# MiZhenxing/Switch-NeRF

Measured on AMD Instinct MI355X. Metric: train rays/sec (8192-ray batch, 256 samples, 8 experts), higher is better.
Workload: dtype bf16; 1 GPU; configs[1]: 8-expert top-1 expertmlp, capacity_factor=1.0, BPR, 8192 rays x 256 samples per step over 1 GPU(s) (8192 rays per GPU), 16 segments of 131072 points per GPU, building.yaml shapes, random-init weights, gate_scale=1.0; global_batch_rays=8192, rays_per_gpu=8192, samples=256, segment_points=131072, parallelism=dp1

## Files before the change

### include/swn.h

```cpp
#ifndef SWN_H
#define SWN_H
#include <stddef.h>
#include <stdint.h>

#ifdef __cplusplus
extern "C" {
#endif

#define SWN_F32 0
#define SWN_BF16 1
#define SWN_F16 2

const char* swn_last_error(void);
int swn_version(void);
int swn_half_dtype(void);

int swn_mfma_probe(int32_t* out, void* stream);

int swn_sample_pe(const float* rays, const float* t_steps, const float* perturb_rand, float perturb,
                  int n_rays, int n_samples, int l_xyz, int l_dir, int dtype,
                  float* z_out, void* pe_xyz, int pe_stride, void* pe_dir, int dir_stride, void* stream);

#define SWN_RNG_UNIFORM 0
#define SWN_RNG_NORMAL 1
// ... 233 lines not shown
  const float* comb_dsig;
  const float* comb_wsig;
  const float* comb_gate;
  float* comb_dgate;
  float* comb_dwsig;
  float* comb_dwsig_ws;
  const float* heads_ws;
  const float* heads_bs;
  const float* heads_wc;
  const float* heads_bc;
  const float* heads_noise;
  float* heads_raw;
  int32_t* sched;
  int32_t x_features;
  int32_t x_k;
  int32_t head_layers;
  int32_t tail_first;
  int32_t y_features;
  const float* tail_gate;
  const int32_t* tail_dropped;
  const int32_t* tail_n_dropped;
  int32_t tail_dropped_max;
  int32_t tail_tokens;
  const int32_t* tail_bias_row;
  swn_chain_layer layers[SWN_MAX_CHAIN_LAYERS];
  int32_t packed_rows;
} swn_chain_desc;

int swn_mlp_chain(const swn_chain_desc* desc, void* stream);
size_t swn_chain_dwsig_workspace_bytes(int n_groups, int group_rows_clamp);
// ... 163 lines not shown
```

### switch_nerf_amd/_lib.py

```python
from __future__ import annotations

import ctypes as C
import os

_HERE = os.path.dirname(os.path.abspath(__file__))
LIB_PATH = os.environ.get("SWN_LIB") or os.path.join(_HERE, "libswn_hip.so")
LIB_PATH_F16 = os.path.join(_HERE, "libswn_hip_f16.so")

F32, BF16, F16 = 0, 1, 2


def source_hash() -> str:
    import hashlib
    h = hashlib.sha256()
    files = [os.path.join(_HERE, "csrc", f) for f in sorted(os.listdir(os.path.join(_HERE, "csrc")))]
    files += [os.path.join(os.path.dirname(_HERE), "include", "swn.h"), os.path.join(_HERE, "build.sh")]
    for f in files:
        if os.path.isfile(f):
            h.update(os.path.basename(f).encode() + b"\0")
            h.update(open(f, "rb").read())
    return h.hexdigest()

vp, i32, i64, f32, sz, u64 = C.c_void_p, C.c_int, C.c_long, C.c_float, C.c_size_t, C.c_uint64

# ... 20 lines not shown
    _fields_ = [("n_levels", i32), ("log2_table", i32), ("base_res", i32), ("per_level_scale", f32), ("aabb_lo", f32 * 3),
                ("aabb_hi", f32 * 3)]


class Camera(C.Structure):
    _fields_ = [("c2w", f32 * 12), ("fx", f32), ("fy", f32), ("cx", f32), ("cy", f32), ("W", C.c_int32), ("H", C.c_int32),
                ("center_pixels", C.c_int32), ("reserved", C.c_int32), ("image_index", C.c_int64)]


class ChainDesc(C.Structure):
    _fields_ = [("dtype", i32), ("n_layers", i32), ("n_groups", i32), ("n_wsets", i32), ("group_stride", i32),
                ("group_rows", vp), ("group_rows_clamp", i32), ("group_begin", vp), ("x", vp), ("x_gather", vp), ("x_save", vp), ("x_scale", vp), ("x_relu", i32),
                ("y", vp), ("y_add", vp), ("y_add_gather", vp), ("geometry", i32), ("tag", i32),
                ("comb_y", vp), ("comb_dsig", vp), ("comb_wsig", vp), ("comb_gate", vp), ("comb_dgate", vp), ("comb_dwsig", vp), ("comb_dwsig_ws", vp),
                ("heads_ws", vp), ("heads_bs", vp), ("heads_wc", vp), ("heads_bc", vp), ("heads_noise", vp), ("heads_raw", vp), ("sched", vp), ("x_features", i32),
                ("x_k", i32), ("head_layers", i32), ("tail_first", i32), ("y_features", i32), ("tail_gate", vp), ("tail_dropped", vp), ("tail_n_dropped", vp),
                ("tail_dropped_max", i32), ("tail_tokens", i32), ("tail_bias_row", vp),
                ("layers", ChainLayer * 12), ("packed_rows", i32)]


SIGNATURES = {
    "swn_version": [],
    "swn_mfma_probe": [vp, vp],
    "swn_sample_pe": [vp, vp, vp, f32, i32, i32, i32, i32, i32, vp, vp, i32, vp, i32, vp],
    "swn_sample_pe_rng": [vp, vp, u64, vp, i64, f32, i32, i32, i32, i32, i32, vp, vp, i32, vp, i32, vp],
    "swn_rng_fill": [vp, i64, i64, i32, f32, u64, vp, i32, vp],
    "swn_rng_fill_rows": [vp, i64, i64, i64, vp, i64, i32, f32, u64, vp, i32, i32, vp],
    "swn_rng_advance": [vp, vp],
    "swn_pe_from_z": [vp, vp, i32, i32, i32, i32, vp, i32, vp],
    "swn_sample_pdf": [vp, vp, vp, i32, i32, i32, vp, vp],
    "swn_cascade_resample": [vp, vp, vp, i32, i32, i32, vp, vp, vp],
# ... 180 lines not shown
```

### switch_nerf_amd/csrc/chain.hip

```cpp
#include "common.hpp"

#ifndef SWN_WIDE
#define SWN_WIDE 0
#endif
#ifndef SWN_CONCAT
#define SWN_CONCAT 0
#endif
#if SWN_WIDE == 2
#define SWN_NS swn_wide2
#elif SWN_WIDE
#define SWN_NS swn_wide
#elif SWN_CONCAT
#define SWN_NS swn_cat
#else
#define SWN_NS swn
#endif
#define SWN_AUX (SWN_WIDE || SWN_CONCAT)
#ifndef SWN_STATIC_EPI
#define SWN_STATIC_EPI 1
#endif
#if defined(SWN_EXP_TIMING) && (!SWN_AUX || SWN_WIDE == 2)
#define SWN_TIMING_ON 1
#else
#define SWN_TIMING_ON 0
// ... 1154 lines not shown
  SWN_CHECK(!d.comb_dwsig == !d.comb_dwsig_ws && (!d.comb_dwsig || (d.head_layers > 0 && d.comb_y && d.comb_dsig)),
            "swn_mlp_chain: comb_dwsig and comb_dwsig_ws come together, with the combine backward of a fused backward chain (head_layers > 0, comb_y, comb_dsig)");
  SWN_CHECK(d.tag != 8 || d.head_layers > 0, "swn_mlp_chain: tag 8 is the expert backward chain behind the tail's backward layers (head_layers > 0)");
  SWN_CHECK(d.tail_first == 0 || (d.geometry == 7 && d.tag == 7), "swn_mlp_chain: a fused tail (tail_first > 0) runs on geometry 7 with tag 7");
  SWN_CHECK(d.tag != 7 || d.tail_first > 0, "swn_mlp_chain: tag 7 is the fused-tail forward chain (tail_first > 0)");
  SWN_CHECK(d.x_features == 0 || d.x_features == d.layers[0].k || (d.x_features == 128 && d.layers[0].k == 256 && d.geometry >= 6),
            "swn_mlp_chain: x_features = %d: only 128-feature rows under a zero-padded k = 256 first layer on geometry 6 / 7", d.x_features);
  if (d.x_k != 0) {
    SWN_CHECK(d.x_k > 0 && d.x_k <= 256, "swn_mlp_chain: x_k = %d not in (0, 256]", d.x_k);
    SWN_CHECK(d.x_k % 16 == 0, "swn_mlp_chain: x_k = %d is not a multiple of the K step (16)", d.x_k);
    SWN_CHECK(d.geometry >= 6, "swn_mlp_chain: x_k = %d: only the persistent chains (geometry 6 / 7) take a real K, not geometry %d", d.x_k, d.geometry);
    SWN_CHECK(d.x_features == 128, "swn_mlp_chain: x_k = %d needs x_features = 128 (a first layer zero-padded in K), not %d", d.x_k, d.x_features);
    SWN_CHECK(d.x_k <= ((d.x_features + 15) & ~15), "swn_mlp_chain: x_k = %d beyond x_features = %d", d.x_k, d.x_features);
    SWN_CHECK(d.tail_first == 0, "swn_mlp_chain: x_k = %d: a fused tail's chain input is 256 features wide", d.x_k);
  }
  SWN_CHECK(!(wide && concat), "swn_mlp_chain: concat-skip layers are built for the 256-feature kernels only");
  SWN_CHECK(d.geometry >= 0 && d.geometry <= 7, "swn_mlp_chain: geometry %d not in [0,7]", d.geometry);
  SWN_CHECK(d.packed_rows >= 0, "swn_mlp_chain: packed_rows %d < 0", d.packed_rows);
  if (d.packed_rows > 0) {
    SWN_CHECK(d.group_begin != nullptr, "swn_mlp_chain: packed mask slots (packed_rows > 0) address the groups through group_begin");
    SWN_CHECK(d.geometry <= 1 || d.geometry == 7, "swn_mlp_chain: packed mask slots (packed_rows > 0) run on geometry 0 / 1 or 7, not %d",
              d.geometry);
  }
  if (d.comb_y && d.head_layers == 0) {
    const int nl = d.layers[d.n_layers - 1].n;
    SWN_CHECK(d.comb_gate && d.comb_dgate, "swn_mlp_chain: combine backward needs comb_gate and comb_dgate");
    SWN_CHECK((nl == 128 || nl == 256 || nl == 512) && nl * (d.dtype == SWN_F32 ? 4 : 2) <= 1024,
              "swn_mlp_chain: combine backward: last layer of 128 / 256 / 512 features, at most 1 KiB per row");
    SWN_CHECK((d.geometry < 2 || d.geometry >= 6) && (d.tag & 0xFF) == 5,
              "swn_mlp_chain: combine backward runs on the 64-row kernels (geometry 0 / 1) or the persistent ones (6 / 7), tag 5");
// ... 21 lines not shown
```

### switch_nerf_amd/csrc/chain_big.hip

```cpp
#include "common.hpp"

namespace swn_big {
using namespace swn;

typedef __attribute__((ext_vector_type(8))) short bf16x8_t;
typedef __attribute__((ext_vector_type(8))) _Float16 f16x8_t;
typedef __attribute__((ext_vector_type(4))) float f32x4_t;
typedef __attribute__((ext_vector_type(16))) float f32x16_t;
typedef __attribute__((ext_vector_type(4))) uint32_t u32x4_t;
typedef __attribute__((ext_vector_type(2))) uint32_t u32x2_t;
typedef __attribute__((ext_vector_type(2))) _Float16 f16x2_t;
#define SWN_LDS(p) ((__attribute__((address_space(3))) void*)(p))
#define SWN_GLB(p) ((const __attribute__((address_space(1))) void*)(p))

constexpr int ROWB = 512;
constexpr int SLOT_B = 8192;
constexpr int NSLOT = 3;
constexpr int KSTEPS = 16;

template <int NW_, int MI_> struct Geo {
  static constexpr int NW = NW_, MI = MI_;
  static constexpr int RG = NW / 4;
  static constexpr int BM = RG * MI * 32;
  static constexpr int NT = NW * 64;
// ... 523 lines not shown
    SWN_MM(1, 1);
    SWN_PIN();
    SWN_MM(2, 0);
    SWN_PIN();
    SWN_MM(2, 1);
    SWN_PIN();
    SWN_MM(3, 0);
    SWN_PIN();
    SWN_MM(3, 1);
#undef SWN_MM
    SWN_PIN();
  }
}
#endif

template <typename E, int RELU, bool BIAS, bool SKIP, typename HOOK>
__device__ __forceinline__ void epilogue_p(f32x16_t (&acc)[4][2], const Ctx& cx, u32x4_t& mk, int bias_off, HOOK hook) {
  typedef G256 G;
  char* smem = cx.smem;
  uint32_t e_base = cx.e_base, e2_base = cx.e2_base;
  asm volatile("" : "+v"(e_base), "+v"(e2_base));
  f32x4_t bias[2][4];
  if constexpr (BIAS) {
#pragma unroll
    for (int ni = 0; ni < 2; ++ni)
#pragma unroll
      for (int g4 = 0; g4 < 4; ++g4)
        bias[ni][g4] = *(const f32x4_t*)(smem + G::BIAS0 + bias_off + (((cx.w & 3) * 64 + 32 * ni + 8 * g4 + 4 * cx.lhi) << 2));
  }
#pragma unroll
// ... 640 lines not shown
      SWN_PIN();
#pragma unroll
      for (int g = 0; g < 4; g += 2) {
        auto r0 = __builtin_amdgcn_permlane32_swap(pp[g * 2], pp[(g + 1) * 2], false, false);
        auto r1 = __builtin_amdgcn_permlane32_swap(pp[g * 2 + 1], pp[(g + 1) * 2 + 1], false, false);
        const u32x4_t o = {(uint32_t)r0[0], (uint32_t)r1[0], (uint32_t)r0[1], (uint32_t)r1[1]};
        *(u32x4_t*)(smem + (e2_base ^ (uint32_t)((4 * ni + g) << 4)) + mi * (32 * ROWB)) = o;
      }
      SWN_PIN();
      if constexpr (hook_halves<HOOK>::value) hook(t);
      else if (t & 1) hook(t >> 1);
    }
  }
}

template <typename E, typename PRE>
__device__ __forceinline__ void write_rows128_tok(const Ctx& cx, void* y, uint32_t oob, const float* wc, int idx_off, int rows, bool heads, PRE pre,
                                                  u32x4_t (&keep)[16]) {
  char* smem = cx.smem;
  const int* idx = (const int*)(smem + idx_off);
  const int l15 = cx.lane & 15, rq = cx.lane >> 4;
  const int rbase = 128 * (cx.w >> 2) + 2 * (cx.w & 3) + 8 * (rq >> 1) + (rq & 1);
  const __amdgpu_buffer_rsrc_t rs = uniform_rsrc(y ? y : (void*)wc, y ? (int)oob : 0);
  f32x4_t w[3][2];
  if (heads) {
#pragma unroll
    for (int c = 0; c < 3; ++c)
#pragma unroll
      for (int q = 0; q < 2; ++q) w[c][q] = *(const f32x4_t*)(smem + T_WC + ((c * 128 + l15 * 8 + 4 * q) << 2));
  }
// ... 25 lines not shown
        a += __int_as_float(__builtin_amdgcn_update_dpp(0, __float_as_int(a), 0x4E, 0xF, 0xF, true));
        a += __int_as_float(__builtin_amdgcn_update_dpp(0, __float_as_int(a), 0x141, 0xF, 0xF, true));
        a += __int_as_float(__builtin_amdgcn_update_dpp(0, __float_as_int(a), 0x140, 0xF, 0xF, true));
        if (l15 == c) ((float*)(smem + T_COL))[c * 256 + rbase + 16 * i] = a;
      }
    }
  }
}

__device__ __forceinline__ int fresh_lane() {
  int l;
  asm volatile("v_mbcnt_lo_u32_b32 %0, -1, 0\n\tv_mbcnt_hi_u32_b32 %0, -1, %0" : "=v"(l));
  return l;
}

template <typename E, int TAG, bool BIAS_INIT, int XS>
__device__ __forceinline__ void chainq_body(const ArgsQ& args) {
  extern __shared__ __attribute__((aligned(16))) char smem[];
  typedef G256 G;
  constexpr int BM = G::BM, MI = 4;
  constexpr bool TAIL = TAG == 7;
  constexpr bool HEAD = TAG == 8;
  constexpr bool DROPS = TAIL || HEAD;
  const swn_chain_desc& d = args.d;
  Ctx cx;
  cx.smem = smem;
  const int tid = threadIdx.x;
  cx.lane = tid & 63;
  cx.w = __builtin_amdgcn_readfirstlane(tid >> 6);
  cx.l31 = cx.lane & 31;
  cx.lhi = cx.lane >> 5;
// ... 27 lines not shown
  auto claim = [&]() -> int {
    int q = 0;
    if (d.sched) {
      const int sq = cur_sq();
      if (fresh_lane() == 0) q = __hip_atomic_fetch_add(d.sched + ((xq + sq) & 7), 1, __ATOMIC_RELAXED, __HIP_MEMORY_SCOPE_AGENT);
    }
    return q;
  };
  auto next_queue = [&]() -> bool {
    int m = 0;
    int sq = cur_sq();
    const int bit = 1 << ((xq + sq) & 7);
    if (fresh_lane() == 0) m = __hip_atomic_fetch_or(d.sched + 9, bit, __ATOMIC_RELAXED, __HIP_MEMORY_SCOPE_AGENT) | bit;
    m = __builtin_amdgcn_readfirstlane(m);
    do { ++sq; } while (sq < 8 && ((m >> ((xq + sq) & 7)) & 1));
    if (fresh_lane() == 0) *(volatile int*)(gcount + 2) = sq;
    return sq < 8;
  };
  auto grab = [&](int slot, int ticket) {
    int vb, g = 0, tile = 0, rows_valid = 0;
    bool first = true;
    int n_groups = d.n_groups, tpg = args.tiles_per_group, n_wsets = d.n_wsets;
    asm volatile("" : "+s"(n_groups), "+s"(tpg), "+s"(n_wsets));
    for (;;) {
      int q;
      if (d.sched) {
        q = first ? ticket : claim();
        first = false;
        q = __builtin_amdgcn_readfirstlane(q);
        const int xs = (xq + cur_sq()) & 7;
        if (args.n_queues != 8) vb = q;
// ... 90 lines not shown
    if (lt < 128) {
      const int r = 128 * rg + lt;
      const long gr = t.grow0 + (r < t.rows ? r : 0);
      if ((TAIL && t.l0) || (HEAD && t.l1 < n_layers)) src = d.tail_dropped[gr];
      else src = d.x_gather ? d.x_gather[gr] : (int)gr;
    }
    return src;
  };
  auto store_row = [&](int src, int idx_off) {
    const int lt = fg * 64 + fresh_lane();
    if (lt < 128) ((int*)(smem + idx_off))[128 * rg + lt] = src < 0 ? 0 : src;
  };
  const bool narrow = d.x_features == 128;
  constexpr bool k_short = XS != KSTEPS;
  static_assert(!k_short || !TAIL, "a fused tail's chain input is 256 features wide");
  auto wrs = [&](int L, int wset) -> __amdgpu_buffer_rsrc_t {
    const int bytes = 8 * (d.layers[L].k >> 4) * 1024;
    const char* p = (const char*)d.layers[L].w + (size_t)wset * bytes;
    return uniform_rsrc(p, bytes);
  };
  auto ws_of = [&](int L, const Tile& t) -> int {
    return ((TAIL && L >= d.tail_first) || (HEAD && L < d.head_layers)) ? 0 : t.wset;
  };
  auto out_rs = [&](void* base, const Tile& t) -> __amdgpu_buffer_rsrc_t {
    return uniform_rsrc((char*)base + t.grow0 * ROWB, t.rows * ROWB);
  };
  u32x4_t wq[WQD][2];
  auto preload_w = [&](int L, int wset, int lane_) {
    const __amdgpu_buffer_rsrc_t r = wrs(L, wset);
#pragma unroll
    for (int ks = 0; ks < WQA; ++ks)
#pragma unroll
      for (int i = 0; i < 2; ++i) wq[ks][i] = __builtin_amdgcn_raw_buffer_load_b128(r, lane_ * 16, ((2 * fg + i) * (d.layers[L].k >> 4) + ks) * 1024, 0);
  };
  auto stage_bias = [&](int L, int wset, int slot) {
    const float* b = d.layers[L].b;
    if (b) {
      const __amdgpu_buffer_rsrc_t rb = uniform_rsrc(b + (size_t)wset * 256, 1024);
      __builtin_amdgcn_raw_ptr_buffer_load_lds(rb, SWN_LDS(smem + G::BIAS0 + slot * 1024 + fg * 256), 4, fresh_lane() * 4, fg * 256, 0, 0);
    } else if constexpr (BIAS_INIT) {
      *(float*)(smem + G::BIAS0 + slot * 1024 + fg * 256 + fresh_lane() * 4) = 0.f;
    }
  };
  auto load_mask = [&](int L, int vb) -> u32x4_t {
    const swn_chain_layer& l_ = d.layers[L];
    if (l_.relu == 2) return *(const u32x4_t*)(l_.mask + ((size_t)(vb * G::NW + cx.w) * 64 + fresh_lane()) * 4);
    return u32x4_t{0u, 0u, 0u, 0u};
  };
  constexpr bool bias_init = BIAS_INIT;
  f32x4_t bv[2][4];
  auto load_bv = [&](int slot) {
    if constexpr (BIAS_INIT) {
      const int lh_ = fresh_lane() >> 5;
#pragma unroll
      for (int ni = 0; ni < 2; ++ni)
#pragma unroll
        for (int g4 = 0; g4 < 4; ++g4)
          bv[ni][g4] = *(const f32x4_t*)(smem + G::BIAS0 + slot * 1024 + ((fg * 64 + 32 * ni + 8 * g4 + 4 * lh_) << 2));
    }
  };

  for (int i = ((int)(blockIdx.x >> 3) & 15) * args.stagger; i > 0; --i) __builtin_amdgcn_s_sleep(16);
  const int yf = TAIL ? (d.y_features ? d.y_features : 256) : 256;
  const uint32_t oob_y = (uint32_t)d.tail_tokens * (uint32_t)(yf * 2), oob_s = (uint32_t)d.tail_tokens * (uint32_t)ROWB;
  auto tail_out = [&](const Ctx& c_, const Tile& t, int idx_off, u32x4_t (&keep)[16]) {
    const bool hd = d.heads_raw != nullptr;
    const int r = 128 * (c_.w >> 2) + 8 * (c_.l31 >> 1) + 2 * (c_.w & 3) + (c_.l31 & 1);
    const bool fin = hd && c_.lhi == 0 && r < t.rows;
// ... 136 lines not shown
      if constexpr (HEAD) {
        if (cur.l1 == n_layers && lts < 128) {
          ((float*)(smem + T_GATE))[128 * rgs + lts] = gate_v;
          ((float*)(smem + T_DSIG))[128 * rgs + lts] = dsig_v;
        }
      }
    }
    if (rg == 0 && it == 0) { stage_bias(cur.l0, ws_of(cur.l0, cur), 0); SWN_WAIT_VM(0); }
    u32x4_t mk_next = load_mask(cur.l0, cur.vb);
    SWN_PIN();
    preload_w(cur.l0, ws_of(cur.l0, cur), fresh_lane());
    SWN_PIN();
    SWN_TM(const long long s1 = TICK(); tS += s1 - s0;)
    Tile nxt = cur;
    const int l_end = HEAD ? cur.l1 : n_layers;
    auto run_layer = [&](const int L, auto first_c) {
      constexpr bool SHORT_K = decltype(first_c)::value;
      const swn_chain_layer& ly = d.layers[L];
      const bool last = L + 1 == l_end;
      load_bv(bc % 3);
      SWN_PIN();
      SWN_WAIT_LGKM0();
      __builtin_amdgcn_s_barrier();
      u32x4_t mk = mk_next;
      if (last) nxt = read_tile((it + 1) & 1);
      {
        SWN_TM(const long long k0 = TICK();)
        const __amdgpu_buffer_rsrc_t rs_cur = wrs(L, ws_of(L, cur));
        if (rg == 0) {
          if (!last) stage_bias(L + 1, ws_of(L + 1, cur), (bc + 1) % 3);
          else if (nxt.vb >= 0) stage_bias(nxt.l0, ws_of(nxt.l0, nxt), (bc + 1) % 3);
        }
        if constexpr (bias_init) {
#pragma unroll
          for (int mi = 0; mi < MI; ++mi)
#pragma unroll
            for (int ni = 0; ni < 2; ++ni)
#pragma unroll
              for (int r = 0; r < 16; ++r) acc[mi][ni][r] = bv[ni][r >> 2][r & 3];
        } else {
#pragma unroll
          for (int mi = 0; mi < MI; ++mi)
#pragma unroll
            for (int ni = 0; ni < 2; ++ni)
#pragma unroll
              for (int r = 0; r < 16; ++r) acc[mi][ni][r] = 0.f;
        }
        {
          const Ctx ck = phase_ctx(true);
          if constexpr (SHORT_K) k_phase2<E, XS, KSTEPS>(acc, ck, rs_cur, wq);
          else k_phase2<E>(acc, ck, rs_cur, wq);
        }
#pragma unroll
        for (int q_ = 0; q_ < WQD; ++q_)
#pragma unroll
          for (int i_ = 0; i_ < 2; ++i_) asm volatile("" : "=v"(wq[q_][i_]));
        SWN_TM(const long long k1 = TICK();)
        __builtin_amdgcn_s_barrier();
        SWN_TM(const long long k2 = TICK(); tK += k1 - k0; tKb += k2 - k1;)
      }
      {
        SWN_TM(const long long e0 = TICK();)
        const Ctx ce = phase_ctx(false);
        const int rge = ce.w >> 2, fge = ce.w & 3;
        const int lane16e = ce.lane * 16;
// ... 19 lines not shown
          if (lt < 128) { const int r = 128 * rg + lt; yrow = d.y_add_gather[cur.grow0 + (r < cur.rows ? r : 0)]; }
        }
        const bool bias_epi = ly.b != nullptr && !bias_init;
        if (ly.skip) {
          stage_pieces_q<false>(ce, (const char*)d.x, 64 * rge + fge, 16, 4, idx_cur);
          SWN_WAIT_VM(0);
          ++n_skip;
          if (ce.lane == 0) __hip_atomic_fetch_add(&gcount[rge], 1, __ATOMIC_RELAXED, __HIP_MEMORY_SCOPE_WORKGROUP);
          while (__builtin_amdgcn_readfirstlane(__hip_atomic_load(&gcount[rge], __ATOMIC_RELAXED, __HIP_MEMORY_SCOPE_WORKGROUP)) < 4 * n_skip)
            __builtin_amdgcn_s_sleep(2);
          __builtin_amdgcn_fence(__ATOMIC_ACQUIRE, "workgroup");
        }
        const bool gate_l = TAIL && L + 1 == d.tail_first, rb_l = TAIL && last;
        auto run_epi = [&](auto hook) {
          typedef decltype(hook) HK;
          if constexpr (TAIL) {
            if (gate_l) { epilogue_q_gate<E, HK>(acc, ce, d.heads_raw != nullptr, hook); return; }
            if (rb_l) { epilogue_q_rowbias<E, HK>(acc, ce, ly.rowbias, ly.rows_per_bias, d.tail_bias_row, yf, idx_cur, hook); return; }
          }
          epilogue_p_dispatch<E, HK>(acc, ce, mk, ly.relu, bias_epi, ly.skip != 0, (bc % 3) * 1024, hook);
        };
        if (wo) {
          const __amdgpu_buffer_rsrc_t rs = wo_tok ? uniform_rsrc(wo, (int)oob_s) : out_rs(wo, cur);
          auto st = [&](int b) {
#pragma unroll
            for (int j = 0; j < 2; ++j) {
              const int c = c0 + 4 * (2 * b + j);
              if constexpr (DROPS) {
                const int r = 2 * c + ce.lhi;
                const uint32_t ri = wo_tok ? (uint32_t)tk[b & 1][j] : (uint32_t)r;
                const uint32_t off = r < cur.rows ? ri * (uint32_t)ROWB + (uint32_t)(ce.l31 * 16) : oob_s;
// ... 40 lines not shown
          const int lt = fg * 64 + fresh_lane();
          if (lt < 128) ((int*)(smem + ((it & 1) ? Q_YIDX + 1024 : Q_YIDX)))[128 * rg + lt] = yrow;
        }
        SWN_PIN();
        if (wo && !held) asm volatile("" :: "v"(wv[1][0]), "v"(wv[1][1]));
        SWN_PIN();
        SWN_TM(const long long e1 = TICK();)
        if (last) {
          SWN_WAIT_LGKM0();
          __builtin_amdgcn_s_barrier();
        }
        SWN_TM(const long long e2 = TICK(); tE += e1 - e0; tEb += e2 - e1;)
      }
      ++bc;
    };
    if constexpr (k_short) run_layer(cur.l0, std::true_type());
    for (int L = cur.l0 + (k_short ? 1 : 0); L < l_end; ++L) run_layer(L, std::false_type());
    prev = cur;
    cur = nxt;
    ++it;
    if (cur.vb < 0) break;
  }
  Ctx cf = cx;
  cf.lane = fresh_lane();
  cf.l31 = cf.lane & 31;
  cf.lhi = cf.lane >> 5;
  u32x4_t keep[16];
#pragma unroll
  for (int i = 0; i < 16; ++i) keep[i] = u32x4_t{0u, 0u, 0u, 0u};
  if constexpr (TAIL) {
    tail_out(cf, prev, ((it - 1) & 1) ? Q_IDX1 : G::IDX0, keep);
  } else if (HEAD && prev.l1 < n_layers) {
// ... 11 lines not shown
  SWN_KEEP16(keep);
  if (rg == 0) __builtin_amdgcn_s_barrier();
#ifdef SWN_BIG_TIMING
  if (d.y_add_gather && !d.y_add && cx.lane == 0 && blockIdx.x < 512) {
    long long* dbg = (long long*)d.y_add_gather + (long)(cx.w * 512 + blockIdx.x) * 8;
    dbg[0] = tS; dbg[1] = tSw; dbg[2] = tK; dbg[3] = tKb; dbg[4] = tE; dbg[5] = tEb + tSb; dbg[6] = it | (tSi << 16); dbg[7] = TICK() - t_start;
  }
#endif
  finish();
}

template <typename E, int TAG, bool BIAS_INIT>
__global__ __launch_bounds__(512, 2) void chainq_kernel(const ArgsQ args) { chainq_body<E, TAG, BIAS_INIT, KSTEPS>(args); }
template <typename E, int TAG, int XS>
__global__ __launch_bounds__(512, 2) void chainq_xk_kernel(const ArgsQ args) { chainq_body<E, TAG, true, XS>(args); }

}

namespace swn {

bool chain_big_eligible(const swn_chain_desc& d) {
  if (d.dtype != SWN_HALF) return false;
#ifdef SWN_BIG_TIMING
  if (d.x_save || d.x_scale) return false;
#else
  if (d.x_save || d.x_scale || d.y_add_gather) return false;
#endif
  if (d.comb_y) return false;
  for (int l = 0; l < d.n_layers; ++l) {
    const swn_chain_layer& ly = d.layers[l];
// ... 174 lines not shown
    case 7: fn = (const void*)chainq_kernel<HalfT, 7, true>; break;
    case 8: fn = (const void*)chainq_kernel<HalfT, 8, true>; break;
    default: fn = d.geometry == 7 ? (const void*)chainq_kernel<HalfT, 0, true> : (const void*)chainq_kernel<HalfT, 0, false>;
  }
#undef SWN_PICKQ
  if (d.x_k) {
    const int xs = d.x_k >> 4;
    fn = nullptr;
    if (d.geometry == 7 && d.tag == 3 && xs == 5) fn = (const void*)chainq_xk_kernel<HalfT, 3, 5>;
    if (d.geometry == 7 && d.tag == 3 && xs == 8) fn = (const void*)chainq_xk_kernel<HalfT, 3, 8>;
    if (d.geometry == 7 && d.tag == 5 && xs == 8) fn = (const void*)chainq_xk_kernel<HalfT, 5, 8>;
    if (d.geometry == 7 && d.tag == 8 && xs == 8) fn = (const void*)chainq_xk_kernel<HalfT, 8, 8>;
    SWN_CHECK(fn != nullptr, "swn_mlp_chain: x_k = %d on geometry %d, tag %d: built for geometry 7 with tag 3 (x_k = 80, 128), tag 5 and tag 8 (x_k = 128)",
              d.x_k, d.geometry, d.tag);
  }
  hipError_t e = hipFuncSetAttribute(fn, hipFuncAttributeMaxDynamicSharedMemorySize, Q_LDS);
  SWN_CHECK(e == hipSuccess, "hipFuncSetAttribute: %s", hipGetErrorString(e));
  const long dws_rows = d.comb_dwsig_ws ? (long)a.n_vb_e * 8 : 0;
  if (dws_rows) {
    e = fill_u32_async(d.comb_dwsig_ws, 0u, (size_t)dws_rows * 1024, as_stream(stream));
    SWN_CHECK(e == hipSuccess, "swn_mlp_chain: comb_dwsig_ws fill: %s", hipGetErrorString(e));
  }
  void* kargs[] = {(void*)&a};
  e = hipLaunchKernel(fn, dim3((unsigned)grid), dim3(G::NT), kargs, Q_LDS, as_stream(stream));
  SWN_CHECK(e == hipSuccess, "swn_mlp_chain (geometry 6 / 7) launch: %s", hipGetErrorString(e));
  if (dws_rows) {
    int rpb = cdiv(dws_rows, DWSIG_RUNS);
    rpb = (rpb + 7) & ~7;
    const int runs = cdiv(dws_rows, rpb);
    float* run_sums = d.comb_dwsig_ws + dws_rows * 256;
// ... 24 lines not shown
```

### switch_nerf_amd/model.py

```python
from __future__ import annotations

import contextlib
import os
import math
from collections import namedtuple
from typing import Dict, Optional

import numpy as np
import torch

from . import _lib, hier, ops, optim
from .noise import DeviceNoise

BUILDING = dict(model_dim=256, num_experts=8, expert_layers=7, skips=(3,), pos_xyz_dim=12, pos_dir_dim=4,
                appearance_dim=48, appearance_count=10, gate_hidden=256, gate_layers=2, layer2_out=128)


def _ceil_to(x, m):
    return (x + m - 1) // m * m


ShHead = namedtuple("ShHead", "dirs want_coef")
CoefHead = namedtuple("CoefHead", "out inner_sigmoid")

# ... 50 lines not shown


CHECK_FINITE_OWNER_TAIL_ERROR = ("the finite guard (check_finite) is not built for expert parallelism with owner_tail=True: the tail's "
                                 "optimizer state is stepped on the experts' ranks inside the step")


def accumulation_rule(iteration: int, steps: int) -> bool:
    return (int(iteration) + 1) % int(steps) != 0


class SwitchNeRF:
    def __init__(self, cfg: dict = BUILDING, dtype=torch.bfloat16, device="cuda", capacity_factor=1.0,
                 batch_prioritized=True, moe_l_aux_wt=5e-4, lr=5e-4, seed=0, gate_noise=-1.0, kernel_switches=None):
        self.cfg, self.dtype, self.dev = dict(cfg), dtype, torch.device(device)
        self.sw = resolve_kernel_switches()
        self._env_overrides = {k: v for k, v in sorted(os.environ.items()) if k.startswith("SWN_")}
        if kernel_switches:
            self.set_kernel_switches(**kernel_switches)
        if dtype == torch.float16:
            _lib.use_half("f16")
        elif dtype == torch.bfloat16:
            _lib.use_half("bf16")
        self.loss_scaler = LossScaler() if dtype == torch.float16 else None
        self.cf, self.bpr, self.wt, self.lr = capacity_factor, batch_prioritized, moe_l_aux_wt, lr
        self.gate_noise, self.gate_noise_draw = float(gate_noise), None
        self.base_lr = lr
        spec = self._configure(cfg)
        if self.affine or self.sh_deg is not None:
            self.sw.update(fused_heads=False, fused_tail=False, fused_tail_bwd=False)
        self.spec, off = {}, 0
# ... 623 lines not shown
            c["drop_begin"], c["dropped"] = o.route_dropped(c["idx"], c["loc"], c["counts"], c["seg_tokens"], self.E, c["cap"])
        w2 = self._l2h_pad(True)
        c["y"] = self._cbuf(c, "y", (P, M), dt) if sv else None
        c["h1"] = self._cbuf(c, "h1", (P, M), dt) if sv else None
        c["h2"] = self._cbuf(c, "h2", (P, H2), dt) if sv else None
        c["raw"] = torch.empty(P, 4, dtype=torch.float32, device=self.dev)
        heads = (self.p["sigma.w"], self.p["sigma.b"], self.p["color.w"], self.p["color.b"], sigma_noise, c["raw"])
        last = layers[-1]
        full = layers[:-1] + [o.Layer(last.w, last.b, relu=last.relu, skip=last.skip, save=c["y"]),
                              o.Layer(self.wf["l1"], self.p["l1.b"].view(1, M), save=c["h1"]),
                              o.Layer(w2, None, relu=1, rowbias=c["c_ray"], rows_per_bias=S)]
        grp, extra = self._group_args(c), dict(group_begin=c.get("group_begin"), packed_rows=c["packed_rows"])

        def run_experts(save=sv):
            o.mlp_chain(c["h0"], full if save else [ly.without_saves() for ly in full], c["h2"] if save else None, tag=7, geometry=7,
                        heads=heads, tail=(L, c["gmax"], c["drop_begin"], c["dropped"], H2), **grp, **extra)
        with self._timed("expert_fwd"):
            run_experts()
        if self.profile:
            def expert_gemm():
                o.mlp_chain(c["h0"], [ly.without_saves() for ly in layers], self._cbuf(c, "eo_probe", (c["rows"], M), dt), tag=1, geometry=7, **grp, **extra)
            c["_relaunch"] = {"expert_fwd": run_experts, "expert_fwd_nosave": lambda: run_experts(False), "expert_gemm_nosave": expert_gemm}
        return c

    def _experts_forward_local(self, c, layers):
        o = ops
        c["row_of_tok"] = c["tok2row"]
        grp = self._group_args(c)

        def run_experts(lys=layers):
            o.mlp_chain(c["h0"], lys, c["eo"], tag=1, geometry=c["geom"], group_begin=c.get("group_begin"), packed_rows=c["packed_rows"], **grp)
# ... 713 lines not shown
```

### switch_nerf_amd/ops.py

```python
from __future__ import annotations

import math
import os

import ctypes as C
from typing import List, Optional, Sequence

import torch

from . import _lib
from ._lib import BF16, F16, F32, ChainDesc, WgradItem, WgradJob, call


def _code(dtype) -> int:
    if dtype == torch.float32:
        return F32
    if dtype == torch.bfloat16:
        if _lib.half_kind() != "bf16":
            raise RuntimeError("bfloat16 tensor, but the fp16 build of the library is selected (_lib.use_half('bf16') first)")
        return BF16
    if dtype == torch.float16:
        if _lib.half_kind() != "f16":
            raise RuntimeError("float16 tensor, but the bf16 build of the library is selected (_lib.use_half('f16') first)")
        return F16
# ... 1201 lines not shown


def chain_mask_words(dtype, n_groups: int, group_stride: int, max_width: int = 256) -> int:
    return int(_lib.load().swn_chain_mask_words(_code(dtype), int(n_groups), int(group_stride), int(max_width)))


def chain_mask_words_packed(dtype, rows: int, n_groups: int, max_width: int = 256) -> int:
    w = C.c_int64(0)
    call("swn_chain_mask_words_packed", _code(dtype), int(rows), int(n_groups), int(max_width), C.byref(w))
    return int(w.value)


def mlp_chain(x, layers: Sequence[Layer], y, n_groups=1, n_wsets=1, group_stride=None, group_rows=None,
              group_rows_clamp=None, x_gather=None, x_save=None, y_add=None, y_add_gather=None, tag=0, x_scale=None,
              x_relu=False, geometry=0, group_begin=None, combine=None, heads=None, sched=None, x_features=0, tail=None, head=None,
              packed_rows=0, x_k=0):
    d = ChainDesc()
    d.packed_rows = int(packed_rows)
    d.dtype = _dt(x)
    d.tag = int(tag)
    d.geometry = int(geometry)
    d.n_layers = len(layers)
    d.n_groups, d.n_wsets = int(n_groups), int(n_wsets)
    d.group_stride = int(group_stride if group_stride is not None else (y if y is not None else heads[5]).shape[0])
    if tail is not None:
        t_first, t_gate, t_begin, t_dropped, t_yf = tail[:5]
        if len(tail) > 5 and tail[5] is not None:
            assert tail[5].dtype == torch.int32 and tail[5].is_contiguous() and tail[5].numel() >= t_gate.numel()
            d.tail_bias_row = _p(tail[5])
        assert t_gate.dtype == torch.float32 and t_begin.dtype == torch.int32 and t_dropped.dtype == torch.int32 and x_gather is not None
        d.tail_first, d.y_features, d.tail_gate, d.tail_dropped = int(t_first), int(t_yf), _p(t_gate), _p(t_dropped)
# ... 1 lines not shown
        d.tail_dropped_max, d.tail_tokens = int(t_dropped.numel()), int(t_gate.numel())
    if head is not None:
        h_layers, h_begin, h_dropped = head
        assert h_begin.dtype == torch.int32 and h_dropped.dtype == torch.int32 and x_gather is not None and combine is not None
        d.head_layers, d.tail_dropped = int(h_layers), _p(h_dropped)
        d.tail_n_dropped = h_begin.data_ptr() + 4 * (h_begin.numel() - 1)
        d.tail_dropped_max, d.tail_tokens = int(h_dropped.numel()), int(x.shape[0])
    d.group_rows = _p(group_rows)
    d.group_rows_clamp = int(group_rows_clamp if group_rows_clamp is not None else d.group_stride)
    d.group_begin = _p(group_begin)
    d.x, d.x_gather, d.x_save, d.y = _p(x), _p(x_gather), _p(x_save), _p(y)
    d.x_scale, d.x_relu = _p(x_scale), int(bool(x_relu))
    d.y_add, d.y_add_gather = _p(y_add), _p(y_add_gather)
    d.x_features = int(x_features)
    d.x_k = int(x_k)
    if sched is None and d.geometry >= 6 and not CHAINQ_STATIC:
        sched = chain_sched(x.device, d.tag)
    if sched is not None:
        assert sched.dtype == torch.int32 and sched.numel() >= 16
        d.sched = _p(sched)
    if combine is not None:
        cy, cds, cws, cg, cdg = combine[:5]
        assert cy.dtype == x.dtype and (cy.shape == y.shape or head is not None) and cg.dtype == torch.float32 and cdg.dtype == torch.float32
        d.comb_y, d.comb_dsig, d.comb_wsig, d.comb_gate, d.comb_dgate = _p(cy), _p(cds), _p(cws), _p(cg), _p(cdg)
        if len(combine) > 5 and combine[5] is not None:
            dws = combine[5]
            assert head is not None and dws.dtype == torch.float32 and dws.numel() == 256 and dws.is_contiguous()
            if packed_rows > 0:
                nb = int(_lib.load().swn_chain_dwsig_workspace_bytes(1, int(packed_rows) + 256 * int(n_groups)))
            else:
# ... 291 lines not shown
```

Baseline: 647,200 rays/s.

## Run fused tail's last expert layer at its real 128-wide N

Adds a specialized kernel variant for the fused-tail forward chain where the last layer computes only the 128 real output columns instead of a zero-padded 256. It adds a narrow K-phase (one MFMA column tile per wave), a narrow bias/rowbias epilogue, and adjusted weight preloading, and moves one schedule counter into LDS for this variant. This is meant to halve the MFMA work and weight traffic of that last layer, at the cost of another kernel instantiation and a different wave work split. It is enabled by default through a switch.

Result: no change. 652,700 rays/s (median of 6 runs) (+0.8%).

```diff
diff --git a/include/swn.h b/include/swn.h
--- a/include/swn.h
+++ b/include/swn.h
@@ -271,6 +271,7 @@
   int32_t* sched;
   int32_t x_features;
   int32_t x_k;
+  int32_t tail_n;
   int32_t head_layers;
   int32_t tail_first;
   int32_t y_features;
diff --git a/switch_nerf_amd/_lib.py b/switch_nerf_amd/_lib.py
--- a/switch_nerf_amd/_lib.py
+++ b/switch_nerf_amd/_lib.py
@@ -58,7 +58,7 @@
                 ("y", vp), ("y_add", vp), ("y_add_gather", vp), ("geometry", i32), ("tag", i32),
                 ("comb_y", vp), ("comb_dsig", vp), ("comb_wsig", vp), ("comb_gate", vp), ("comb_dgate", vp), ("comb_dwsig", vp), ("comb_dwsig_ws", vp),
                 ("heads_ws", vp), ("heads_bs", vp), ("heads_wc", vp), ("heads_bc", vp), ("heads_noise", vp), ("heads_raw", vp), ("sched", vp), ("x_features", i32),
-                ("x_k", i32), ("head_layers", i32), ("tail_first", i32), ("y_features", i32), ("tail_gate", vp), ("tail_dropped", vp), ("tail_n_dropped", vp),
+                ("x_k", i32), ("tail_n", i32), ("head_layers", i32), ("tail_first", i32), ("y_features", i32), ("tail_gate", vp), ("tail_dropped", vp), ("tail_n_dropped", vp),
                 ("tail_dropped_max", i32), ("tail_tokens", i32), ("tail_bias_row", vp),
                 ("layers", ChainLayer * 12), ("packed_rows", i32)]
 
diff --git a/switch_nerf_amd/csrc/chain.hip b/switch_nerf_amd/csrc/chain.hip
--- a/switch_nerf_amd/csrc/chain.hip
+++ b/switch_nerf_amd/csrc/chain.hip
@@ -1192,6 +1192,13 @@
     SWN_CHECK(d.x_k <= ((d.x_features + 15) & ~15), "swn_mlp_chain: x_k = %d beyond x_features = %d", d.x_k, d.x_features);
     SWN_CHECK(d.tail_first == 0, "swn_mlp_chain: x_k = %d: a fused tail's chain input is 256 features wide", d.x_k);
   }
+  if (d.tail_n != 0) {
+    SWN_CHECK(d.tail_first > 0 && d.geometry == 7 && d.tag == 7,
+              "swn_mlp_chain: tail_n = %d: only the fused forward (tail_first > 0, geometry 7, tag 7) runs its last layer at a real N, not geometry %d, tag %d",
+              d.tail_n, d.geometry, d.tag);
+    SWN_CHECK(d.tail_n == 128 && d.y_features == 128, "swn_mlp_chain: tail_n = %d under y_features = %d: built for 128 real outputs of 256 only",
+              d.tail_n, d.y_features);
+  }
   SWN_CHECK(!(wide && concat), "swn_mlp_chain: concat-skip layers are built for the 256-feature kernels only");
   SWN_CHECK(d.geometry >= 0 && d.geometry <= 7, "swn_mlp_chain: geometry %d not in [0,7]", d.geometry);
   SWN_CHECK(d.packed_rows >= 0, "swn_mlp_chain: packed_rows %d < 0", d.packed_rows);
diff --git a/switch_nerf_amd/csrc/chain_big.hip b/switch_nerf_amd/csrc/chain_big.hip
--- a/switch_nerf_amd/csrc/chain_big.hip
+++ b/switch_nerf_amd/csrc/chain_big.hip
@@ -561,6 +561,55 @@
 }
 #endif
 
+template <typename E, int AD = 4>
+__device__ __forceinline__ void k_phase_n(f32x16_t (&acc)[4][2], const Ctx& cx, __amdgpu_buffer_rsrc_t rs_cur, u32x4_t (&wq)[WQD][2]) {
+  constexpr int MI = 4, NS = KSTEPS, AA = AD - 1;
+  static_assert(WQA >= 1 && WQA <= 4 && AA >= 1 && AA <= 3 && NS > AA && NS > WQA, "k_phase_n: counted waits");
+  char* smem = cx.smem;
+  const int lane16 = cx.lane * 16;
+  const int fg = cx.w & 3;
+  u32x4_t fa[AD][MI];
+  uint32_t a_base = cx.a_base;
+  asm volatile("" : "+v"(a_base));
+  auto read_a = [&](int ks, int mi) {
+    fa[ks % AD][mi] = *(const u32x4_t*)(smem + (a_base ^ (uint32_t)(ks << 5)) + mi * (32 * ROWB));
+  };
+  auto load_w = [&](int ks) { wq[ks % WQD][0] = __builtin_amdgcn_raw_buffer_load_b128(rs_cur, lane16, (fg * NS + ks) * 1024, 0); };
+#pragma unroll
+  for (int s = 0; s < AA; ++s)
+#pragma unroll
+    for (int mi = 0; mi < MI; ++mi) read_a(s, mi);
+#pragma unroll
+  for (int ks = 0; ks < NS; ++ks) {
+    {
+      const int younger = (NS - 1 - ks < WQA - 1 ? NS - 1 - ks : WQA - 1) + (ks < WQA ? WQA - ks : 0);
+      if (younger >= 6) SWN_WAIT_VM(6); else if (younger == 5) SWN_WAIT_VM(5); else if (younger == 4) SWN_WAIT_VM(4);
+      else if (younger == 3) SWN_WAIT_VM(3); else if (younger == 2) SWN_WAIT_VM(2); else if (younger == 1) SWN_WAIT_VM(1); else SWN_WAIT_VM(0);
+    }
+    {
+      const int younger = (NS - 1 - ks < AA - 1 ? NS - 1 - ks : AA - 1) * 4;
+      if (younger >= 8) SWN_WAIT_LGKM(8); else if (younger == 4) SWN_WAIT_LGKM(4); else SWN_WAIT_LGKM(0);
+    }
+    SWN_PIN();
+#define SWN_MM(mi) acc[mi][0] = E::mfma(wq[ks % WQD][0], fa[ks % AD][mi], acc[mi][0])
+    SWN_MM(0);
+    SWN_PIN();
+    if (ks + AA < NS) { read_a(ks + AA, 0); read_a(ks + AA, 1); }
+    SWN_PIN();
+    SWN_MM(1);
+    SWN_PIN();
+    if (ks + AA < NS) { read_a(ks + AA, 2); read_a(ks + AA, 3); }
+    SWN_PIN();
+    SWN_MM(2);
+    SWN_PIN();
+    if (ks + WQA < NS) load_w(ks + WQA);
+    SWN_PIN();
+    SWN_MM(3);
+#undef SWN_MM
+    SWN_PIN();
+  }
+}
+
 template <typename E, int RELU, bool BIAS, bool SKIP, typename HOOK>
 __device__ __forceinline__ void epilogue_p(f32x16_t (&acc)[4][2], const Ctx& cx, u32x4_t& mk, int bias_off, HOOK hook) {
   typedef G256 G;
@@ -1231,6 +1280,57 @@
   }
 }
 
+template <typename E, typename HOOK>
+__device__ __forceinline__ void epilogue_q_rowbias_n(f32x16_t (&acc)[4][2], const Ctx& cx, const float* rowbias, int rpb, const int32_t* bias_row,
+                                                     int idx_off, HOOK hook) {
+  constexpr int NF = 128;
+  char* smem = cx.smem;
+  const int fg = cx.w & 3;
+  uint32_t e2_base = cx.e2_base ^ (uint32_t)((fg << 7) ^ (fg << 6));
+  asm volatile("" : "+v"(e2_base));
+  const int row0 = 128 * (cx.w >> 2) + cx.l31;
+  const float* rb[4];
+#pragma unroll
+  for (int mi = 0; mi < 4; ++mi) {
+    const uint32_t tok = (uint32_t)((const int*)(smem + idx_off))[row0 + 32 * mi];
+    const uint32_t br = bias_row ? (uint32_t)bias_row[tok] : tok / (uint32_t)rpb;
+    rb[mi] = rowbias ? rowbias + (size_t)br * NF + fg * 32 + 4 * cx.lhi : nullptr;
+  }
+  f32x4_t bq[2][4];
+  auto fetch = [&](int mi) {
+#pragma unroll
+    for (int g4 = 0; g4 < 4; ++g4)
+#ifdef SWN_ABL_NORB
+      bq[mi & 1][g4] = f32x4_t{0.f, 0.f, 0.f, 0.f};
+#else
+      bq[mi & 1][g4] = rb[mi] ? *(const f32x4_t*)(rb[mi] + 8 * g4) : f32x4_t{0.f, 0.f, 0.f, 0.f};
+#endif
+  };
+  fetch(0);
+#pragma unroll
+  for (int mi = 0; mi < 4; ++mi) {
+    if (mi + 1 < 4) fetch(mi + 1);
+    uint32_t pp[8];
+#pragma unroll
+    for (int k = 0; k < 8; ++k) {
+      const int g4 = k >> 1, i = k & 1;
+      pp[k] = pk_relu16(E::pack2(acc[mi][0][g4 * 4 + 2 * i] + bq[mi & 1][g4][2 * i], acc[mi][0][g4 * 4 + 2 * i + 1] + bq[mi & 1][g4][2 * i + 1]));
+    }
+    SWN_PIN();
+    if constexpr (hook_halves<HOOK>::value) hook(2 * mi);
+#pragma unroll
+    for (int g = 0; g < 4; g += 2) {
+      auto r0 = __builtin_amdgcn_permlane32_swap(pp[g * 2], pp[(g + 1) * 2], false, false);
+      auto r1 = __builtin_amdgcn_permlane32_swap(pp[g * 2 + 1], pp[(g + 1) * 2 + 1], false, false);
+      const u32x4_t o = {(uint32_t)r0[0], (uint32_t)r1[0], (uint32_t)r0[1], (uint32_t)r1[1]};
+      *(u32x4_t*)(smem + (e2_base ^ (uint32_t)(g << 4)) + mi * (32 * ROWB)) = o;
+    }
+    SWN_PIN();
+    if constexpr (hook_halves<HOOK>::value) hook(2 * mi + 1);
+    else hook(mi);
+  }
+}
+
 template <typename E, typename PRE>
 __device__ __forceinline__ void write_rows128_tok(const Ctx& cx, void* y, uint32_t oob, const float* wc, int idx_off, int rows, bool heads, PRE pre,
                                                   u32x4_t (&keep)[16]) {
@@ -1286,7 +1386,7 @@
   return l;
 }
 
-template <typename E, int TAG, bool BIAS_INIT, int XS>
+template <typename E, int TAG, bool BIAS_INIT, int XS, bool TN = false>
 __device__ __forceinline__ void chainq_body(const ArgsQ& args) {
   extern __shared__ __attribute__((aligned(16))) char smem[];
   typedef G256 G;
@@ -1344,7 +1444,10 @@
     if (fresh_lane() == 0) m = __hip_atomic_fetch_or(d.sched + 9, bit, __ATOMIC_RELAXED, __HIP_MEMORY_SCOPE_AGENT) | bit;
     m = __builtin_amdgcn_readfirstlane(m);
     do { ++sq; } while (sq < 8 && ((m >> ((xq + sq) & 7)) & 1));
-    if (fresh_lane() == 0) *(volatile int*)(gcount + 2) = sq;
+    if (fresh_lane() == 0) {
+      if constexpr (TN) *(volatile __attribute__((address_space(3))) int*)SWN_LDS(gcount + 2) = sq;
+      else *(volatile int*)(gcount + 2) = sq;
+    }
     return sq < 8;
   };
   auto grab = [&](int slot, int ticket) {
@@ -1465,6 +1568,7 @@
   const bool narrow = d.x_features == 128;
   constexpr bool k_short = XS != KSTEPS;
   static_assert(!k_short || !TAIL, "a fused tail's chain input is 256 features wide");
+  static_assert(!TN || (TAIL && BIAS_INIT), "the last layer at its real N: the fused tail on geometry 7");
   auto wrs = [&](int L, int wset) -> __amdgpu_buffer_rsrc_t {
     const int bytes = 8 * (d.layers[L].k >> 4) * 1024;
     const char* p = (const char*)d.layers[L].w + (size_t)wset * bytes;
@@ -1479,10 +1583,20 @@
   u32x4_t wq[WQD][2];
   auto preload_w = [&](int L, int wset, int lane_) {
     const __amdgpu_buffer_rsrc_t r = wrs(L, wset);
-#pragma unroll
-    for (int ks = 0; ks < WQA; ++ks)
-#pragma unroll
-      for (int i = 0; i < 2; ++i) wq[ks][i] = __builtin_amdgcn_raw_buffer_load_b128(r, lane_ * 16, ((2 * fg + i) * (d.layers[L].k >> 4) + ks) * 1024, 0);
+    if constexpr (TN) {
+      const int ksn = d.layers[L].k >> 4;
+      const int t0 = L + 1 == n_layers ? fg : 2 * fg, t1 = L + 1 == n_layers ? fg : 2 * fg + 1;
+#pragma unroll
+      for (int ks = 0; ks < WQA; ++ks) {
+        wq[ks][0] = __builtin_amdgcn_raw_buffer_load_b128(r, lane_ * 16, (t0 * ksn + ks) * 1024, 0);
+        wq[ks][1] = __builtin_amdgcn_raw_buffer_load_b128(r, lane_ * 16, (t1 * ksn + ks) * 1024, 0);
+      }
+    } else {
+#pragma unroll
+      for (int ks = 0; ks < WQA; ++ks)
+#pragma unroll
+        for (int i = 0; i < 2; ++i) wq[ks][i] = __builtin_amdgcn_raw_buffer_load_b128(r, lane_ * 16, ((2 * fg + i) * (d.layers[L].k >> 4) + ks) * 1024, 0);
+    }
   };
   auto stage_bias = [&](int L, int wset, int slot) {
     const float* b = d.layers[L].b;
@@ -1500,9 +1614,14 @@
   };
   constexpr bool bias_init = BIAS_INIT;
   f32x4_t bv[2][4];
-  auto load_bv = [&](int slot) {
+  auto load_bv = [&](int slot, auto narrow_c) {
     if constexpr (BIAS_INIT) {
       const int lh_ = fresh_lane() >> 5;
+      if constexpr (decltype(narrow_c)::value) {
+#pragma unroll
+        for (int g4 = 0; g4 < 4; ++g4) bv[0][g4] = *(const f32x4_t*)(smem + G::BIAS0 + slot * 1024 + ((fg * 32 + 8 * g4 + 4 * lh_) << 2));
+        return;
+      }
 #pragma unroll
       for (int ni = 0; ni < 2; ++ni)
 #pragma unroll
@@ -1669,11 +1788,12 @@
     SWN_TM(const long long s1 = TICK(); tS += s1 - s0;)
     Tile nxt = cur;
     const int l_end = HEAD ? cur.l1 : n_layers;
-    auto run_layer = [&](const int L, auto first_c) {
+    auto run_layer = [&](const int L, auto first_c, auto narrow_c) {
       constexpr bool SHORT_K = decltype(first_c)::value;
+      constexpr bool NARROW_N = decltype(narrow_c)::value;
       const swn_chain_layer& ly = d.layers[L];
-      const bool last = L + 1 == l_end;
-      load_bv(bc % 3);
+      const bool last = TN ? NARROW_N : L + 1 == l_end;
+      load_bv(bc % 3, narrow_c);
       SWN_PIN();
       SWN_WAIT_LGKM0();
       __builtin_amdgcn_s_barrier();
@@ -1690,7 +1810,7 @@
 #pragma unroll
           for (int mi = 0; mi < MI; ++mi)
 #pragma unroll
-            for (int ni = 0; ni < 2; ++ni)
+            for (int ni = 0; ni < (NARROW_N ? 1 : 2); ++ni)
 #pragma unroll
               for (int r = 0; r < 16; ++r) acc[mi][ni][r] = bv[ni][r >> 2][r & 3];
         } else {
@@ -1704,6 +1824,7 @@
         {
           const Ctx ck = phase_ctx(true);
           if constexpr (SHORT_K) k_phase2<E, XS, KSTEPS>(acc, ck, rs_cur, wq);
+          else if constexpr (NARROW_N) k_phase_n<E>(acc, ck, rs_cur, wq);
           else k_phase2<E>(acc, ck, rs_cur, wq);
         }
 #pragma unroll
@@ -1753,7 +1874,10 @@
         const bool gate_l = TAIL && L + 1 == d.tail_first, rb_l = TAIL && last;
         auto run_epi = [&](auto hook) {
           typedef decltype(hook) HK;
-          if constexpr (TAIL) {
+          if constexpr (NARROW_N) {
+            epilogue_q_rowbias_n<E, HK>(acc, ce, ly.rowbias, ly.rows_per_bias, d.tail_bias_row, idx_cur, hook);
+            return;
+          } else if constexpr (TAIL) {
             if (gate_l) { epilogue_q_gate<E, HK>(acc, ce, d.heads_raw != nullptr, hook); return; }
             if (rb_l) { epilogue_q_rowbias<E, HK>(acc, ce, ly.rowbias, ly.rows_per_bias, d.tail_bias_row, yf, idx_cur, hook); return; }
           }
@@ -1824,8 +1948,9 @@
       }
       ++bc;
     };
-    if constexpr (k_short) run_layer(cur.l0, std::true_type());
-    for (int L = cur.l0 + (k_short ? 1 : 0); L < l_end; ++L) run_layer(L, std::false_type());
+    if constexpr (k_short) run_layer(cur.l0, std::true_type(), std::false_type());
+    for (int L = cur.l0 + (k_short ? 1 : 0); L < l_end - (TN ? 1 : 0); ++L) run_layer(L, std::false_type(), std::false_type());
+    if constexpr (TN) run_layer(l_end - 1, std::false_type(), std::true_type());
     prev = cur;
     cur = nxt;
     ++it;
@@ -1867,6 +1992,11 @@
 __global__ __launch_bounds__(512, 2) void chainq_kernel(const ArgsQ args) { chainq_body<E, TAG, BIAS_INIT, KSTEPS>(args); }
 template <typename E, int TAG, int XS>
 __global__ __launch_bounds__(512, 2) void chainq_xk_kernel(const ArgsQ args) { chainq_body<E, TAG, true, XS>(args); }
+template <typename E, int TN>
+__global__ __launch_bounds__(512, 2) void chainq_tn_kernel(const ArgsQ args) {
+  static_assert(TN == 128, "the last tail layer at its real N: 128 of 256");
+  chainq_body<E, 7, true, KSTEPS, true>(args);
+}
 
 }
 
@@ -2071,6 +2201,12 @@
     SWN_CHECK(fn != nullptr, "swn_mlp_chain: x_k = %d on geometry %d, tag %d: built for geometry 7 with tag 3 (x_k = 80, 128), tag 5 and tag 8 (x_k = 128)",
               d.x_k, d.geometry, d.tag);
   }
+  if (d.tail_n) {
+    fn = nullptr;
+    if (d.geometry == 7 && d.tag == 7 && d.tail_first > 0 && d.tail_n == 128 && d.y_features == 128) fn = (const void*)chainq_tn_kernel<HalfT, 128>;
+    SWN_CHECK(fn != nullptr, "swn_mlp_chain: tail_n = %d on geometry %d, tag %d, y_features %d: built for tail_n = y_features = 128 on the fused forward (geometry 7, tag 7)",
+              d.tail_n, d.geometry, d.tag, d.y_features);
+  }
   hipError_t e = hipFuncSetAttribute(fn, hipFuncAttributeMaxDynamicSharedMemorySize, Q_LDS);
   SWN_CHECK(e == hipSuccess, "hipFuncSetAttribute: %s", hipGetErrorString(e));
   const long dws_rows = d.comb_dwsig_ws ? (long)a.n_vb_e * 8 : 0;
diff --git a/switch_nerf_amd/model.py b/switch_nerf_amd/model.py
--- a/switch_nerf_amd/model.py
+++ b/switch_nerf_amd/model.py
@@ -88,6 +88,7 @@
                  batch_prioritized=True, moe_l_aux_wt=5e-4, lr=5e-4, seed=0, gate_noise=-1.0, kernel_switches=None):
         self.cfg, self.dtype, self.dev = dict(cfg), dtype, torch.device(device)
         self.sw = resolve_kernel_switches()
+        self.sw["tail_n"] = os.environ.get("SWN_TAIL_N", "1") != "0"
         self._env_overrides = {k: v for k, v in sorted(os.environ.items()) if k.startswith("SWN_")}
         if kernel_switches:
             self.set_kernel_switches(**kernel_switches)
@@ -741,7 +742,8 @@
 
         def run_experts(save=sv):
             o.mlp_chain(c["h0"], full if save else [ly.without_saves() for ly in full], c["h2"] if save else None, tag=7, geometry=7,
-                        heads=heads, tail=(L, c["gmax"], c["drop_begin"], c["dropped"], H2), **grp, **extra)
+                        heads=heads, tail=(L, c["gmax"], c["drop_begin"], c["dropped"], H2), tail_n=H2 if self.sw["tail_n"] else 0,
+                        **grp, **extra)
         with self._timed("expert_fwd"):
             run_experts()
         if self.profile:
diff --git a/switch_nerf_amd/ops.py b/switch_nerf_amd/ops.py
--- a/switch_nerf_amd/ops.py
+++ b/switch_nerf_amd/ops.py
@@ -1239,7 +1239,7 @@
 def mlp_chain(x, layers: Sequence[Layer], y, n_groups=1, n_wsets=1, group_stride=None, group_rows=None,
               group_rows_clamp=None, x_gather=None, x_save=None, y_add=None, y_add_gather=None, tag=0, x_scale=None,
               x_relu=False, geometry=0, group_begin=None, combine=None, heads=None, sched=None, x_features=0, tail=None, head=None,
-              packed_rows=0, x_k=0):
+              packed_rows=0, x_k=0, tail_n=0):
     d = ChainDesc()
     d.packed_rows = int(packed_rows)
     d.dtype = _dt(x)
@@ -1271,6 +1271,7 @@
     d.y_add, d.y_add_gather = _p(y_add), _p(y_add_gather)
     d.x_features = int(x_features)
     d.x_k = int(x_k)
+    d.tail_n = int(tail_n)
     if sched is None and d.geometry >= 6 and not CHAINQ_STATIC:
         sched = chain_sched(x.device, d.tag)
     if sched is not None:
```
